# octree-nn/octfusion

Measured on AMD Instinct MI355X. Metric: denoising-steps/sec (depth-8 octree, batch 8), higher is better.
Workload: dtype f32 storage, fp16x3 products (fp16 hi + lo operand pairs = 22 significand bits, three fp16 MFMAs per product, fp32 accumulate)

## Files before the change

octfusion_amd/csrc/ofx_gemm.hip:

```cpp
#include "ofx_gemm_common.h"

constexpr int BM = 128;
constexpr int BK = 32;
constexpr int A_LD = BK + 4;
constexpr int MODE_DENSE = 0;
constexpr int MODE_GATHER = 1;

struct TileCoords { int split, tm, tn; };
__device__ __forceinline__ TileCoords tile_coords(const GemmArgs& g) {
  const int ntile = g.ntm * g.ntn;
  int bid = ofx_xcd_swizzle(blockIdx.x, ntile * g.nsplit);
  const int split = bid / ntile;
  bid -= split * ntile;
  const int tm = bid / g.ntn;
  return {split, tm, bid - tm * g.ntn};
}

__device__ __forceinline__ void load_a_dense(const GemmArgs& g, int64_t m0, int64_t k0, float4 (&va)[4]) {
  const int c4 = threadIdx.x & 7, r0 = threadIdx.x >> 3;
  const int64_t k = k0 + c4 * 4;
  const bool vec = ((g.lda & 3) == 0) && (k + 3 < g.K) && ((((uintptr_t)g.A) & 15) == 0);
#pragma unroll
  for (int i = 0; i < 4; ++i) {
    const int64_t m = m0 + r0 + 32 * i;
// ... 389 lines not shown
  const int tpd = MODE == MODE_DENSE ? nkt_all : g.cin / BK;
  const int nkt_g = MODE == MODE_DENSE ? nkt_all : ndir * tpd;
  const int g_begin = kt_begin < nkt_g ? kt_begin : nkt_g;
  const int g_end = kt_end < nkt_g ? kt_end : nkt_g;
  const int t_begin = kt_begin > nkt_g ? kt_begin : nkt_g;

  int64_t m_0 = m0 + r0, m_1 = m_0 + 32, m_2 = m_0 + 64, m_3 = m_0 + 96;
  const int64_t mmax = g.M - 1;
  m_0 = m_0 < mmax ? m_0 : mmax; m_1 = m_1 < mmax ? m_1 : mmax;
  m_2 = m_2 < mmax ? m_2 : mmax; m_3 = m_3 < mmax ? m_3 : mmax;
  const gip t0 = tab + m_0 * ndir;
  const gip t1 = tab + m_1 * ndir;
  const gip t2 = tab + m_2 * ndir;
  const gip t3 = tab + m_3 * ndir;
  int64_t dr0 = m_0, dr1 = m_1, dr2 = m_2, dr3 = m_3;
  if (MODE == MODE_DENSE && g.a_rows) { dr0 = g.a_rows[m_0]; dr1 = g.a_rows[m_1]; dr2 = g.a_rows[m_2]; dr3 = g.a_rows[m_3]; }
  const gfp dp0 = xp + dr0 * ldx, dp1 = xp + dr1 * ldx, dp2 = xp + dr2 * ldx, dp3 = xp + dr3 * ldx;
  const int kclamp = (int)g.K - 4;

  int64_t bcol[NI];
#pragma unroll
  for (int j = 0; j < NI; ++j) {
    int64_t nn = n0 + (wn * NI + j) * 32 + l31;
    bcol[j] = (nn < Ncols ? nn : Ncols - 1) + (int64_t)h * Ncols;
  }
  char* const a_st = smem8 + (r0 * 80 + c4 * 8);
  const char* const a_ld = smem8 + ((wm * MI * 32 + l31) * 80 + 16 * h);

  struct BFrag { u32x4 h[2][NI], l[2][NI]; };
  struct RegSet { float4 a0, a1, a2, a3; };
  struct IdxSet { uint32_t i0, i1, i2, i3; };

  auto load_bfrag = [&](int ktw, BFrag& F) {
    const gqp wk = w16 + (int64_t)ktw * 4 * Ncols;
#pragma unroll
    for (int c = 0; c < 2; ++c)
#pragma unroll
      for (int j = 0; j < NI; ++j) {
        F.h[c][j] = wk[(int64_t)(2 * c) * Ncols + bcol[j]];
        F.l[c][j] = wk[lo_off + (int64_t)(2 * c) * Ncols + bcol[j]];
      }
  };
  auto store_a = [&](int buf, const RegSet& R) {
    char* a = a_st + buf * BUF_BYTES;
    uint2 hi, lo;
    split16x4<H16>(R.a0, hi, lo);
    *reinterpret_cast<uint2*>(a) = hi; *reinterpret_cast<uint2*>(a + A_BYTES) = lo;
    split16x4<H16>(R.a1, hi, lo);
    *reinterpret_cast<uint2*>(a + 32 * 80) = hi; *reinterpret_cast<uint2*>(a + 32 * 80 + A_BYTES) = lo;
    split16x4<H16>(R.a2, hi, lo);
    *reinterpret_cast<uint2*>(a + 64 * 80) = hi; *reinterpret_cast<uint2*>(a + 64 * 80 + A_BYTES) = lo;
    split16x4<H16>(R.a3, hi, lo);
    *reinterpret_cast<uint2*>(a + 96 * 80) = hi; *reinterpret_cast<uint2*>(a + 96 * 80 + A_BYTES) = lo;
  };
  auto compute = [&](int buf, const BFrag& F) {
    const char* a = a_ld + buf * BUF_BYTES;
    u32x4h ah[2][MI], al[2][MI];
#pragma unroll
    for (int c = 0; c < 2; ++c)
#pragma unroll
      for (int i = 0; i < MI; ++i) {
        ah[c][i] = *reinterpret_cast<const u32x4h*>(a + i * 32 * 80 + 32 * c);
        al[c][i] = *reinterpret_cast<const u32x4h*>(a + i * 32 * 80 + 32 * c + A_BYTES);
      }
#pragma unroll
    for (int c = 0; c < 2; ++c) {
#pragma unroll
      for (int i = 0; i < MI; ++i)
#pragma unroll
        for (int j = 0; j < NI; ++j)
          acc[i][j] = mfma16<H16>(al[c][i], F.h[c][j], acc[i][j]);
#pragma unroll
      for (int i = 0; i < MI; ++i)
#pragma unroll
        for (int j = 0; j < NI; ++j)
          acc[i][j] = mfma16<H16>(ah[c][i], F.l[c][j], acc[i][j]);
#pragma unroll
      for (int i = 0; i < MI; ++i)
#pragma unroll
        for (int j = 0; j < NI; ++j)
          acc[i][j] = mfma16<H16>(ah[c][i], F.h[c][j], acc[i][j]);
    }
  };

  if (g_begin < g_end) {
    RegSet R0, R1;
    IdxSet I0 = {0, 0, 0, 0}, I1 = {0, 0, 0, 0};
    BFrag F0, F1;
    auto clampg = [&](int it) { return it < nkt_g ? it : nkt_g - 1; };
    auto ktw_of = [&](int it) {
      const int itc = clampg(it);
      return MODE == MODE_DENSE ? itc : (itc % ndir) * tpd + itc / ndir;
    };
    auto load_idx = [&](int it, IdxSet& I) {
      if (MODE == MODE_DENSE) return;
      const int dc = clampg(it) % ndir;
      I.i0 = (uint32_t)t0[dc]; I.i1 = (uint32_t)t1[dc]; I.i2 = (uint32_t)t2[dc]; I.i3 = (uint32_t)t3[dc];
    };
    auto load_rows = [&](int it, const IdxSet& I, RegSet& R) {
      const int itc = clampg(it);
      if (MODE == MODE_DENSE) {
        int cc = itc * BK + c4 * 4;
        cc = cc < kclamp ? cc : kclamp;
        R.a0 = ldg4(dp0 + cc); R.a1 = ldg4(dp1 + cc); R.a2 = ldg4(dp2 + cc); R.a3 = ldg4(dp3 + cc);
      } else {
        const int cc = (itc / ndir) * BK + c4 * 4;
        R.a0 = ldg4(xp + src_off(I.i0, ldx, n_src, aux_delta) + cc);
        R.a1 = ldg4(xp + src_off(I.i1, ldx, n_src, aux_delta) + cc);
        R.a2 = ldg4(xp + src_off(I.i2, ldx, n_src, aux_delta) + cc);
        R.a3 = ldg4(xp + src_off(I.i3, ldx, n_src, aux_delta) + cc);
      }
    };
    auto load_bchunk = [&](int ktw, int c, BFrag& F) {
      const gqp wk = w16 + (int64_t)ktw * 4 * Ncols + (int64_t)(2 * c) * Ncols;
#pragma unroll
      for (int j = 0; j < NI; ++j) { F.h[c][j] = wk[bcol[j]]; F.l[c][j] = wk[lo_off + bcol[j]]; }
    };
    auto store_half = [&](int buf, const float4& v0, const float4& v1, int row_off) {
      char* a = a_st + buf * BUF_BYTES + row_off * 80;
      uint2 hi, lo;
      split16x4<H16>(v0, hi, lo);
      *reinterpret_cast<uint2*>(a) = hi; *reinterpret_cast<uint2*>(a + A_BYTES) = lo;
      split16x4<H16>(v1, hi, lo);
      *reinterpret_cast<uint2*>(a + 32 * 80) = hi; *reinterpret_cast<uint2*>(a + 32 * 80 + A_BYTES) = lo;
    };
#define OFX_FENCE() __builtin_amdgcn_sched_barrier(0)
    auto step = [&](int it, int buf, const IdxSet& Iuse, IdxSet& Iload, const BFrag& Fcur, BFrag& Fnext,
                    RegSet& Rnew, const RegSet& Rold) {
      const char* a = a_ld + buf * BUF_BYTES;
      const int ktw = ktw_of(it + 1);
      u32x4h ah[2][MI], al[2][MI];
#pragma unroll
      for (int c = 0; c < 2; ++c)
#pragma unroll
        for (int i = 0; i < MI; ++i) {
          ah[c][i] = *reinterpret_cast<const u32x4h*>(a + i * 32 * 80 + 32 * c);
          al[c][i] = *reinterpret_cast<const u32x4h*>(a + i * 32 * 80 + 32 * c + A_BYTES);
        }
      load_idx(it + 3, Iload);
      OFX_FENCE();
#define OFX_MFMA_GROUP(AOP, BOP, C)                                                                        \
      _Pragma("unroll") for (int i = 0; i < MI; ++i)                                                        \
        _Pragma("unroll") for (int j = 0; j < NI; ++j)                                                      \
          acc[i][j] = mfma16<H16>(AOP[C][i], Fcur.BOP[C][j], acc[i][j]);
      OFX_MFMA_GROUP(al, h, 0);
      OFX_FENCE();
      load_bchunk(ktw, 0, Fnext);
      OFX_FENCE();
      OFX_MFMA_GROUP(ah, l, 0);
      OFX_FENCE();
      load_bchunk(ktw, 1, Fnext);
      OFX_FENCE();
      OFX_MFMA_GROUP(ah, h, 0);
      OFX_FENCE();
      load_rows(it + 2, Iuse, Rnew);
      OFX_FENCE();
      OFX_MFMA_GROUP(al, h, 1);
      OFX_FENCE();
      store_half(buf ^ 1, Rold.a0, Rold.a1, 0);
      OFX_FENCE();
      OFX_MFMA_GROUP(ah, l, 1);
      OFX_FENCE();
      store_half(buf ^ 1, Rold.a2, Rold.a3, 64);
      OFX_FENCE();
      OFX_MFMA_GROUP(ah, h, 1);
#undef OFX_MFMA_GROUP
      __syncthreads();
    };

    load_idx(g_begin, I0);
    load_idx(g_begin + 1, I1);
    OFX_FENCE();
    load_rows(g_begin, I0, R0);
    load_bchunk(ktw_of(g_begin), 0, F0);
    load_bchunk(ktw_of(g_begin), 1, F0);
    OFX_FENCE();
    load_idx(g_begin + 2, I0);
    OFX_FENCE();
    load_rows(g_begin + 1, I1, R1);
    OFX_FENCE();
    store_half(0, R0.a0, R0.a1, 0);
    store_half(0, R0.a2, R0.a3, 64);
    __syncthreads();
    int it = g_begin;
    for (; it + 1 < g_end; it += 2) {
      step(it, 0, I0, I1, F0, F1, R0, R1);
      step(it + 1, 1, I1, I0, F1, F0, R1, R0);
    }
    if (it < g_end) step(it, 0, I0, I1, F0, F1, R0, R1);
    __syncthreads();
#undef OFX_FENCE
  }

  for (int kt = t_begin; kt < kt_end; ++kt) {
    const int cc = (kt - nkt_g) * BK + c4 * 4;
    RegSet R;
    BFrag F;
    R.a0 = ldg4(tfp + m_0 * ldt + cc);
    R.a1 = ldg4(tfp + m_1 * ldt + cc);
    R.a2 = ldg4(tfp + m_2 * ldt + cc);
    R.a3 = ldg4(tfp + m_3 * ldt + cc);
    load_bfrag(kt, F);
    store_a(0, R);
    __syncthreads();
    compute(0, F);
    __syncthreads();
  }

  epilogue_store<WM, WN, MI, NI>(g, acc, m0, n0, wm, wn, l31, h, split);
}

__device__ __forceinline__ uint32_t bf16_rne_bits(float f) {
  const uint32_t u = __float_as_uint(f);
  return (u + 0x7fffu + ((u >> 16) & 1u)) >> 16;
}
__global__ void pack_bf16x3_kernel(const float* __restrict__ Wp, int64_t Kp, int64_t N, uint16_t* __restrict__ W16,
                                   int h16) {
  const int64_t total = Kp * N;
  const float wscale = h16 ? reinterpret_cast<const float*>(W16 + 2 * total)[1] : 1.f;
  for (int64_t t = (int64_t)blockIdx.x * blockDim.x + threadIdx.x; t < total; t += (int64_t)gridDim.x * blockDim.x) {
    const int64_t kg = t / (N * 8), rem = t - kg * N * 8;
    const int64_t n = rem / 8;
    const int kk = (int)(rem - n * 8);
    const int64_t k = kg * 8 + kk;
    const float w = Wp[((k >> 2) * N + n) * 4 + (k & 3)];
    if (h16) {
      const float ws = g2_sat16(w * wscale);
      const _Float16 hi = (_Float16)ws;
      const _Float16 lo = (_Float16)(ws - (float)hi);
      W16[t] = __builtin_bit_cast(unsigned short, hi);
      W16[total + t] = __builtin_bit_cast(unsigned short, lo);
    } else {
      const uint32_t hi = bf16_rne_bits(w);
      const float wl = w - __uint_as_float(hi << 16);
      W16[t] = (uint16_t)hi;
      W16[total + t] = (uint16_t)bf16_rne_bits(wl);
    }
  }
}
static int g_precision = 3;
static int pack_bf16x3(const float* Wp, int64_t Kp, int64_t N, hipStream_t st) {
  uint16_t* W16 = reinterpret_cast<uint16_t*>(const_cast<float*>(Wp) + Kp * N);
  if (ofx_launch_weight_scale(Wp, 1, 0, Kp * N, 1, g_precision == 3 ? 1 : 0, const_cast<float*>(Wp) + 2 * Kp * N, st))
    return OFX_ELAUNCH;
  pack_bf16x3_kernel<<<ofx_grid(Kp * N, 256), 256, 0, st>>>(Wp, Kp, N, W16, g_precision == 3 ? 1 : 0);
  return hipGetLastError() == hipSuccess ? OFX_OK : OFX_ELAUNCH;
}

extern "C" int ofx_set_precision(int mode) {
  if (mode < 0 || mode > 3) return OFX_EINVAL;
  g_precision = mode;
  return OFX_OK;
}
extern "C" int ofx_get_precision(void) { return g_precision; }
extern "C" int64_t ofx_packed_floats(int64_t Kp, int64_t N) { return 2 * Kp * N + 32; }

__global__ void __launch_bounds__(256) multi_mean_kernel(const float* __restrict__ x, int64_t ldx, int cin,
                                                         const int32_t* __restrict__ seg_ptr,
                                                         const int32_t* __restrict__ col,
                                                         const int32_t* __restrict__ multi_seg, int64_t V,
                                                         float* __restrict__ aux, int64_t ldaux,
                                                         const float* __restrict__ w) {
  const int c4n = cin >> 2;
  const int64_t total = (V + 1) * c4n;
  for (int64_t t = (int64_t)blockIdx.x * blockDim.x + threadIdx.x; t < total; t += (int64_t)gridDim.x * blockDim.x) {
    const int64_t v = t / c4n;
    const int c = (int)(t - v * c4n) * 4;
    float4 acc = f4zero();
    if (v > 0) {
      const int64_t s = multi_seg[v - 1];
      const int32_t a = seg_ptr[s], e = seg_ptr[s + 1];
      if (w) {
        for (int32_t p = a; p < e; ++p) {
          const float wp = w[p];
          const float4 xv = *reinterpret_cast<const float4*>(x + (int64_t)col[p] * ldx + c);
          acc.x += wp * xv.x; acc.y += wp * xv.y; acc.z += wp * xv.z; acc.w += wp * xv.w;
        }
      } else {
        for (int32_t p = a; p < e; ++p) f4add(acc, *reinterpret_cast<const float4*>(x + (int64_t)col[p] * ldx + c));
        const float inv = 1.f / (float)(e - a);
        acc.x *= inv; acc.y *= inv; acc.z *= inv; acc.w *= inv;
      }
    }
    *reinterpret_cast<float4*>(aux + v * ldaux + c) = acc;
  }
}

__global__ void __launch_bounds__(256) splitk_reduce_kernel(const GemmArgs g) {
  const int64_t total = g.M * g.N;
  for (int64_t t = (int64_t)blockIdx.x * blockDim.x + threadIdx.x; t < total; t += (int64_t)gridDim.x * blockDim.x) {
    const int64_t m = t / g.N, n = t - m * g.N;
    float v = 0.f;
    for (int s = 0; s < g.nsplit; ++s) v += g.ws[(int64_t)s * total + t];
    if (g.oscale_p) v *= *g.oscale_p;
    if (g.bias) v += g.bias[n];
    if (g.emb) v += g.emb[(int64_t)g.bid[m] * g.lde + n];
    if (g.res) v += g.res[m * g.ldr + n];
    int64_t om = m;
    if (g.out_rows) { om = g.out_rows[m]; if (om < 0) continue; }
    g.out[om * g.ldc + n] = v;
  }
}

__global__ void __launch_bounds__(256) splitk_reduce_v4_kernel(const GemmArgs g) {
  const int64_t n4 = g.N >> 2, total4 = g.M * n4, total = g.M * g.N;
  for (int64_t t = (int64_t)blockIdx.x * blockDim.x + threadIdx.x; t < total4; t += (int64_t)gridDim.x * blockDim.x) {
    const int64_t m = t / n4, n = (t - m * n4) * 4;
    const float* p = g.ws + m * g.N + n;
    float4 v = f4zero();
    int s = 0;
    for (; s + 7 < g.nsplit; s += 8) {
      float4 a[8];
#pragma unroll
      for (int u = 0; u < 8; ++u) a[u] = *reinterpret_cast<const float4*>(p + (int64_t)(s + u) * total);
#pragma unroll
      for (int u = 0; u < 8; ++u) f4add(v, a[u]);
    }
    for (; s + 3 < g.nsplit; s += 4) {
      const float4 a0 = *reinterpret_cast<const float4*>(p + (int64_t)s * total);
      const float4 a1 = *reinterpret_cast<const float4*>(p + (int64_t)(s + 1) * total);
      const float4 a2 = *reinterpret_cast<const float4*>(p + (int64_t)(s + 2) * total);
      const float4 a3 = *reinterpret_cast<const float4*>(p + (int64_t)(s + 3) * total);
      f4add(v, a0); f4add(v, a1); f4add(v, a2); f4add(v, a3);
    }
    for (; s < g.nsplit; ++s) f4add(v, *reinterpret_cast<const float4*>(p + (int64_t)s * total));
    if (g.oscale_p) { const float osc = *g.oscale_p; v.x *= osc; v.y *= osc; v.z *= osc; v.w *= osc; }
    if (g.bias) f4add(v, *reinterpret_cast<const float4*>(g.bias + n));
    if (g.emb) f4add(v, *reinterpret_cast<const float4*>(g.emb + (int64_t)g.bid[m] * g.lde + n));
    if (g.res) f4add(v, *reinterpret_cast<const float4*>(g.res + m * g.ldr + n));
    int64_t om = m;
    if (g.out_rows) { om = g.out_rows[m]; if (om < 0) continue; }
    if (g.out_planes) ofx_store_planes4(g.out, om * g.ldc + n, v, g.out_planes);
    else *reinterpret_cast<float4*>(g.out + om * g.ldc + n) = v;
  }
}

template <void (*KERNEL)(const GemmArgs), size_t LDS>
static int launch_tiled(GemmArgs& g, hipStream_t st) {
  static bool attr_set[OFX_MAX_DEVICES] = {};
  if (LDS > 64 * 1024 &&
      !ofx_raise_lds_limit(reinterpret_cast<const void*>(KERNEL), (int)LDS, attr_set))
    return OFX_ELAUNCH;
  KERNEL<<<g.ntm * g.ntn * g.nsplit, 256, LDS, st>>>(g);
  return OFX_OK;
}
template <int MODE, int WM, int WN, int MI, int NI>
static int launch_cfg(GemmArgs& g, int flavour, hipStream_t st) {
  constexpr size_t lds_f32 = (2 * BM * A_LD + 2 * 8 * (WN * NI * 32) * 4) * sizeof(float);
  constexpr size_t lds_16 = 2 * (2 * BM * 80);
  switch (flavour) {
    case 3: return launch_tiled<gemm_pairs_x3_kernel<MODE, WM, WN, MI, NI, 1>, lds_16>(g, st);
    case 2: return launch_tiled<gemm_pairs_x3_kernel<MODE, WM, WN, MI, NI, 0>, lds_16>(g, st);
    case 1: return launch_tiled<gemm_fast_kernel<MODE, WM, WN, MI, NI>, lds_f32>(g, st);
  }
  if constexpr (MODE == MODE_DENSE) return launch_tiled<gemm_dense_generic_kernel<WM, WN, MI, NI>, lds_f32>(g, st);
  return OFX_EINVAL;
}

__global__ void __launch_bounds__(256) stats_reduce_kernel(const float* __restrict__ part, int64_t nwr, int wr_rows,
                                                            int64_t N, const int32_t* __restrict__ bid,
                                                            double* __restrict__ stats, int64_t stats_ld) {
  __shared__ double red[3][64][2];
  const int c = threadIdx.x & 63, rg = threadIdx.x >> 6;
  const int64_t n = (int64_t)blockIdx.y * 64 + c;
  const int64_t w0 = (int64_t)blockIdx.x * 64;
  const int64_t nc = n < N ? n : N - 1;
  int b[16];
  float2 v[16];
#pragma unroll
  for (int i = 0; i < 16; ++i) {
    const int64_t w = w0 + rg * 16 + i;
    const int64_t wc = w < nwr ? w : nwr - 1;
    b[i] = bid[wc * wr_rows];
    v[i] = *reinterpret_cast<const float2*>(part + (wc * N + nc) * 2);
    if (w >= nwr) { b[i] = -1; v[i] = make_float2(0.f, 0.f); }
  }
  const int bfirst = bid[w0 * wr_rows];
  bool ok = true;
#pragma unroll
  for (int i = 0; i < 16; ++i) ok = ok && (b[i] == bfirst || b[i] < 0);
  const bool uni = __syncthreads_and(ok);
  auto flush = [&](int bb, double s, double q) {
    double* o = stats + ((int64_t)bb * stats_ld + n) * 2;
    unsafeAtomicAdd(o, s); unsafeAtomicAdd(o + 1, q);
  };
  if (uni) {
    double s = 0.0, q = 0.0;
#pragma unroll
    for (int i = 0; i < 16; ++i) { s += (double)v[i].x; q += (double)v[i].y; }
    if (rg > 0) { red[rg - 1][c][0] = s; red[rg - 1][c][1] = q; }
    __syncthreads();
    if (rg == 0 && n < N) {
#pragma unroll
      for (int r = 0; r < 3; ++r) { s += red[r][c][0]; q += red[r][c][1]; }
      flush(bfirst, s, q);
    }
  } else if (n < N) {
    double s = 0.0, q = 0.0;
    int sb = -1;
#pragma unroll
    for (int i = 0; i < 16; ++i) {
      if (b[i] < 0) continue;
      if (b[i] != sb) {
        if (sb >= 0) flush(sb, s, q);
        sb = b[i]; s = 0.0; q = 0.0;
      }
      s += (double)v[i].x; q += (double)v[i].y;
    }
    if (sb >= 0) flush(sb, s, q);
  }
}

int ofx_launch_stats_reduce(const GemmArgs& g, int wr_rows, hipStream_t st) {
  const int64_t nwr = ofx_cdiv(g.M, wr_rows);
  stats_reduce_kernel<<<dim3((unsigned)ofx_cdiv(nwr, 64), (unsigned)ofx_cdiv(g.N, 64)), 256, 0, st>>>(
      g.stats_part, nwr, wr_rows, g.N, g.bid, g.stats, g.stats_ld);
  OFX_LAUNCH_CHECK();
  return OFX_OK;
}

template <int MODE>
static int launch_gemm(GemmArgs& g, float* ws, size_t ws_bytes, hipStream_t st) {
  if (g.M <= 0 || g.N <= 0) return OFX_OK;
  if (MODE == MODE_GATHER && !(g.fast && g.nbr_ext && g.aux && (!g.out_rows || g.gather_out_rows))) return OFX_EINVAL;
  {
    auto al16 = [](const void* p) { return (reinterpret_cast<uintptr_t>(p) & 15) == 0; };
    g.vec4 = g.N % 4 == 0 && al16(g.out) && g.ldc % 4 == 0 && (!g.res || (al16(g.res) && g.ldr % 4 == 0)) &&
             (!g.emb || (al16(g.emb) && g.lde % 4 == 0)) && (!g.bias || al16(g.bias));
  }
  const int bn = g.N <= 32 ? 32 : (g.N <= 64 ? 64 : 128);
  g.ntm = (int)ofx_cdiv(g.M, BM);
  g.ntn = (int)ofx_cdiv(g.N, bn);
  const int nkt = (int)(g.Kp / BK);
  int nsplit = 1;
  const int tiles = g.ntm * g.ntn;
  if (ws && tiles < 256 && nkt >= 8) {
    nsplit = (int)ofx_cdiv(512, tiles);
    if (nsplit > nkt / 4) nsplit = nkt / 4;
    if (nsplit > 64) nsplit = 64;
    const size_t per = (size_t)g.M * g.N * sizeof(float);
    if ((size_t)nsplit * per > ws_bytes) nsplit = (int)(ws_bytes / per);
    if (nsplit < 2) nsplit = 1;
  }
  g.kt_per_split = (int)ofx_cdiv(nkt, nsplit);
  nsplit = (int)ofx_cdiv(nkt, g.kt_per_split);
  g.nsplit = nsplit;
  g.ws = ws;
  bool fast = true;
  if (MODE == MODE_DENSE) {
    fast = ((g.lda & 3) == 0) && ((g.K & 3) == 0) && g.K >= 4 && ((((uintptr_t)g.A) & 15) == 0);
    if (fast) { g.ndir = 1; g.n_src = 0; g.aux = g.A; g.tf = g.A; g.ldt = g.lda; g.nbr_ext = (const int32_t*)g.A; }
  }
  g.W16 = (g_precision != 1) ? reinterpret_cast<const uint16_t*>(g.Wp + g.Kp * g.N) : nullptr;
  const int wr_rows = bn == 32 ? 32 : 64;
  const int64_t nwr = ofx_cdiv(g.M, wr_rows);
  if (!(g.stats && g.vec4 && nsplit == 1 && g.stats_part &&
        (size_t)nwr * g.N * 2 * sizeof(float) <= g.stats_part_bytes && (((uintptr_t)g.stats_part) & 15) == 0))
    g.stats_part = nullptr;
  g.oscale_p = (fast && g.W16) ? g.Wp + 2 * g.Kp * g.N : nullptr;
  const int flavour = !fast ? 0 : (!g.W16 ? 1 : (g_precision == 3 ? 3 : 2));
  int rc;
  if (bn == 32) rc = launch_cfg<MODE, 4, 1, 1, 1>(g, flavour, st);
  else if (bn == 64) rc = launch_cfg<MODE, 2, 2, 2, 1>(g, flavour, st);
  else rc = launch_cfg<MODE, 2, 2, 2, 2>(g, flavour, st);
  if (rc) return rc;
  if (nsplit > 1) {
    const bool ws16 = (((uintptr_t)g.ws) & 15) == 0;
    if (g.vec4 && ws16) splitk_reduce_v4_kernel<<<ofx_grid(g.M * (g.N >> 2), 256), 256, 0, st>>>(g);
    else splitk_reduce_kernel<<<ofx_grid(g.M * g.N, 256), 256, 0, st>>>(g);
  }
  if (g.stats_part) {
    rc = ofx_launch_stats_reduce(g, wr_rows, st);
    if (rc) return rc;
  }
  OFX_LAUNCH_CHECK();
  return OFX_OK;
}

static inline int64_t pad32(int64_t v) { return (v + 31) / 32 * 32; }

extern "C" int64_t ofx_packed_k(int64_t K) { return pad32(K); }
extern "C" int64_t ofx_graphconv_packed_k(int cin, int nt) {
  return pad32(7 * (int64_t)cin) + (nt > 1 ? pad32(7 * (int64_t)nt) : 0);
}

__global__ void pack_weights_kernel(const float* __restrict__ W, int64_t sk, int64_t sn, int64_t K, int64_t N, int cin,
                                    int nt, float* __restrict__ Wp, int64_t Kp) {
  const int64_t total = (Kp / 4) * N;
  const int ntc = nt > 1 ? nt : 0;
  const int64_t Kf = (7 * (int64_t)cin + 31) / 32 * 32;
  for (int64_t t = (int64_t)blockIdx.x * blockDim.x + threadIdx.x; t < total; t += (int64_t)gridDim.x * blockDim.x) {
    const int64_t kq = t / N, n = t - kq * N;
    float v[4];
#pragma unroll
    for (int kk = 0; kk < 4; ++kk) {
      const int64_t k = kq * 4 + kk;
      int64_t src = -1;
      if (cin > 0) {
        if (k < 7 * (int64_t)cin) {
          const int64_t dir = k / cin, c = k - dir * cin;
          src = dir * (cin + ntc) + c;
        } else if (k >= Kf && ntc > 0 && k - Kf < 7 * (int64_t)ntc) {
          const int64_t kt = k - Kf, dir = kt / ntc, ty = kt - dir * ntc;
          src = dir * (cin + ntc) + cin + ty;
        }
      } else if (k < K) {
        src = k;
      }
      v[kk] = src >= 0 ? W[src * sk + n * sn] : 0.f;
    }
    *reinterpret_cast<float4*>(Wp + t * 4) = make_float4(v[0], v[1], v[2], v[3]);
  }
}

extern "C" int ofx_pack_weights(const float* W, int64_t sk, int64_t sn, int64_t K, int64_t N, int cin, int nt,
                                float* Wp, int64_t Kp, void* stream) {
  if (!W || !Wp || K < 1 || N < 1 || (Kp & 31) || cin < 0 || nt < 0) return OFX_EINVAL;
  if (cin > 0) {
    if (Kp != ofx_graphconv_packed_k(cin, nt) || K != 7 * (int64_t)(cin + (nt > 1 ? nt : 0))) return OFX_EINVAL;
  } else if (Kp != pad32(K)) {
    return OFX_EINVAL;
  }
  if (((uintptr_t)Wp & 15) != 0) return OFX_EINVAL;
  pack_weights_kernel<<<ofx_grid((Kp / 4) * N, 256), 256, 0, ofx_stream(stream)>>>(W, sk, sn, K, N, cin, nt, Wp, Kp);
  if (int rc = pack_bf16x3(Wp, Kp, N, ofx_stream(stream))) return rc;
  OFX_LAUNCH_CHECK();
  return OFX_OK;
}

__global__ void pack_conv3d_kernel(const float* __restrict__ W, int cin, int64_t N, float* __restrict__ Wp, int64_t Kp) {
  const int64_t total = (Kp / 4) * N;
  for (int64_t t = (int64_t)blockIdx.x * blockDim.x + threadIdx.x; t < total; t += (int64_t)gridDim.x * blockDim.x) {
    const int64_t kq = t / N, n = t - kq * N;
    float v[4];
#pragma unroll
    for (int kk = 0; kk < 4; ++kk) {
      const int64_t k = kq * 4 + kk;
      float w = 0.f;
      if (k < 27 * (int64_t)cin) {
        const int64_t tap = k / cin, c = k - tap * cin;
        w = W[(n * cin + c) * 27 + tap];
      }
      v[kk] = w;
    }
    *reinterpret_cast<float4*>(Wp + t * 4) = make_float4(v[0], v[1], v[2], v[3]);
  }
}

extern "C" int64_t ofx_conv3d_packed_k(int cin) { return pad32(27 * (int64_t)cin); }

extern "C" int ofx_pack_conv3d(const float* W, int cin, int cout, float* Wp, void* stream) {
  if (!W || !Wp || cin < 1 || cout < 1 || ((uintptr_t)Wp & 15)) return OFX_EINVAL;
  const int64_t Kp = ofx_conv3d_packed_k(cin);
  pack_conv3d_kernel<<<ofx_grid((Kp / 4) * cout, 256), 256, 0, ofx_stream(stream)>>>(W, cin, cout, Wp, Kp);
  if (int rc = pack_bf16x3(Wp, Kp, cout, ofx_stream(stream))) return rc;
  OFX_LAUNCH_CHECK();
  return OFX_OK;
}

extern "C" int ofx_gemm_f32_planes(const float* A, int64_t lda, const int32_t* a_rows, int64_t M, int64_t K,
                                   const float* Wp, int64_t Kp, int64_t N, const float* bias, const float* res, int64_t ldr,
                                   float* out, int64_t ldc, const int32_t* out_rows, void* ws, size_t ws_bytes,
                                   int out_mode, void* stream) {
  if (M == 0 && K >= 1 && N >= 1) return OFX_OK;
  if (M < 0 || K < 1 || N < 1 || !Wp || !out || (M > 0 && !A) || Kp != pad32(K) || lda < K || ldc < N ||
      (res && ldr < N) || ((uintptr_t)Wp & 15))
    return OFX_EINVAL;
  if (out_mode != 0 && out_mode != 2 && out_mode != 3) return OFX_EINVAL;
  if (out_mode && ((N & 3) || (ldc & 31) || ((uintptr_t)out & 127) || (res && ((ldr & 3) || ((uintptr_t)res & 15))) ||
                   (bias && ((uintptr_t)bias & 15)) || ((uintptr_t)ws & 15)))
    return OFX_EINVAL;
  GemmArgs g = {};
  g.A = A; g.lda = lda; g.a_rows = a_rows;
  g.M = M; g.K = K; g.Wp = Wp; g.Kp = Kp; g.N = N; g.bias = bias;
  g.res = res; g.ldr = ldr; g.out = out; g.ldc = ldc; g.out_rows = out_rows; g.out_planes = out_mode;
  return launch_gemm<MODE_DENSE>(g, (float*)ws, ws_bytes, ofx_stream(stream));
}
extern "C" int ofx_gemm_f32(const float* A, int64_t lda, const int32_t* a_rows, int64_t M, int64_t K, const float* Wp,
                            int64_t Kp, int64_t N, const float* bias, const float* res, int64_t ldr, float* out,
                            int64_t ldc, const int32_t* out_rows, void* ws, size_t ws_bytes, void* stream) {
  return ofx_gemm_f32_planes(A, lda, a_rows, M, K, Wp, Kp, N, bias, res, ldr, out, ldc, out_rows, ws, ws_bytes, 0, stream);
}

static int gather_common(GemmArgs& g, const float* x, int64_t ldx, int cin, int ndir, int64_t n_rows,
                         const int32_t* nbr, const int32_t* seg_ptr, const int32_t* col, const float* Wp, int64_t Kp,
                         int cout, const float* bias, const float* emb, int64_t lde, const int32_t* batch_id,
                         const float* res, int64_t ldr, float* out, int64_t ldc) {
  if (n_rows < 0 || cin < 1 || cout < 1 || !x || !nbr || !Wp || !out || ldx < cin || ldc < cout ||
      (res && ldr < cout) || (emb && (!batch_id || lde < cout)) || ((uintptr_t)Wp & 15))
    return OFX_EINVAL;
  g.x = x; g.ldx = ldx; g.cin = cin; g.ndir = ndir;
  g.fast = (cin % 32 == 0) && ((ldx & 3) == 0) && (((uintptr_t)x & 15) == 0);
  g.nbr = nbr; g.seg_ptr = seg_ptr; g.col = col;
  g.Kf = pad32((int64_t)ndir * cin);
  g.M = n_rows; g.K = Kp; g.Wp = Wp; g.Kp = Kp; g.N = cout; g.bias = bias;
  g.emb = emb; g.lde = lde; g.bid = batch_id; g.res = res; g.ldr = ldr; g.out = out; g.ldc = ldc;
  return OFX_OK;
}

__device__ __forceinline__ float gather_elem(const GemmArgs& g, int64_t row, int64_t k) {
  if (k >= (int64_t)g.ndir * g.cin) return 0.f;
  const int dir = (int)(k / g.cin), c = (int)(k - (int64_t)dir * g.cin);
  const int32_t nb = g.nbr[row * g.ndir + dir];
  if (nb >= 0) return g.x[(int64_t)nb * g.ldx + c];
  if (nb == -1) return 0.f;
  const int64_t s = row * g.ndir + dir;
  const int32_t a = g.seg_ptr[s], e = g.seg_ptr[s + 1];
  float acc = 0.f;
  if (g.edge_w) {
    for (int32_t p = a; p < e; ++p) acc += g.edge_w[p] * g.x[(int64_t)g.col[p] * g.ldx + c];
    return acc;
  }
  for (int32_t p = a; p < e; ++p) acc += g.x[(int64_t)g.col[p] * g.ldx + c];
  if (e - a > 1) acc /= (float)(e - a);
  return acc;
}
__global__ void __launch_bounds__(256) col_rows_kernel(const GemmArgs g, int64_t row0, int64_t rows,
                                                       float* __restrict__ colbuf) {
  const int64_t k4n = g.Kp >> 2, total = rows * k4n;
  for (int64_t t = (int64_t)blockIdx.x * blockDim.x + threadIdx.x; t < total; t += (int64_t)gridDim.x * blockDim.x) {
    const int64_t r = t / k4n, k = (t - r * k4n) * 4;
    const int64_t row = row0 + r;
    float v[4];
#pragma unroll
    for (int kk = 0; kk < 4; ++kk)
      v[kk] = (k + kk < g.Kf) ? gather_elem(g, row, k + kk) : g.tf[row * g.ldt + (k + kk - g.Kf)];
    *reinterpret_cast<float4*>(colbuf + t * 4) = make_float4(v[0], v[1], v[2], v[3]);
  }
}

static int launch_gather_via_col(const GemmArgs& g, float* ws, size_t ws_bytes, hipStream_t st) {
  if (!ws || (((uintptr_t)ws) & 15)) return OFX_EINVAL;
  size_t tail = ws_bytes / 8;
  if (tail > (size_t(16) << 20)) tail = size_t(16) << 20;
  tail &= ~size_t(15);
  const size_t row_bytes = (size_t)g.Kp * sizeof(float);
  int64_t chunk = (int64_t)((ws_bytes - tail) / row_bytes) / 128 * 128;
  if (chunk < 128) return OFX_EINVAL;
  float* tail_ws = reinterpret_cast<float*>(reinterpret_cast<char*>(ws) + (ws_bytes - tail));
  for (int64_t r0 = 0; r0 < g.M; r0 += chunk) {
    const int64_t rows = g.M - r0 < chunk ? g.M - r0 : chunk;
    col_rows_kernel<<<ofx_grid(rows * (g.Kp >> 2), 256), 256, 0, st>>>(g, r0, rows, ws);
    GemmArgs d = {};
    d.A = ws; d.lda = g.Kp; d.M = rows; d.K = g.Kp; d.Wp = g.Wp; d.Kp = g.Kp; d.N = g.N; d.bias = g.bias;
    d.emb = g.emb; d.lde = g.lde; d.bid = g.bid ? g.bid + r0 : nullptr;
    d.res = g.res ? g.res + r0 * g.ldr : nullptr; d.ldr = g.ldr;
    d.out = g.out + r0 * g.ldc; d.ldc = g.ldc;
    d.stats = g.stats; d.stats_ld = g.stats_ld;
    if (g.stats) { d.stats_part = tail_ws; d.stats_part_bytes = tail; }
    const int rc = launch_gemm<MODE_DENSE>(d, g.stats ? nullptr : tail_ws, tail, st);
    if (rc) return rc;
  }
  return OFX_OK;
}

extern "C" int ofx_graphconv_fwd(const float* x, int64_t ldx, int cin, int64_t n_nodes, const int32_t* nbr,
                                 const int32_t* seg_ptr, const int32_t* col, const int32_t* nbr_ext,
                                 const int32_t* multi_seg, int64_t n_multi, float* aux, const float* type_frac,
                                 int64_t ldt, int nt_pad, const float* Wp, int64_t Kp, int cout, const float* bias,
                                 const float* emb, int64_t lde, const int32_t* batch_id, const float* res, int64_t ldr,
                                 float* out, int64_t ldc, double* stats, int64_t stats_ld, void* ws, size_t ws_bytes,
                                 void* stream) {
  if (n_nodes == 0 && cin >= 1 && cout >= 1) return OFX_OK;
  GemmArgs g = {};
  int rc = gather_common(g, x, ldx, cin, 7, n_nodes, nbr, seg_ptr, col, Wp, Kp, cout, bias, emb, lde, batch_id, res,
                         ldr, out, ldc);
  if (rc) return rc;
  if (!seg_ptr || !col) return OFX_EINVAL;
  if (nt_pad < 0 || (nt_pad & 31) || Kp != g.Kf + nt_pad) return OFX_EINVAL;
  if (nt_pad > 0 && (!type_frac || ldt < nt_pad || (ldt & 3) || ((uintptr_t)type_frac & 15))) return OFX_EINVAL;
  g.tf = type_frac; g.ldt = ldt;
  if (stats) {
    if (!batch_id || stats_ld < cout) return OFX_EINVAL;
    g.stats = stats; g.stats_ld = stats_ld; g.bid = batch_id;
    g.stats_part = (float*)ws; g.stats_part_bytes = ws_bytes;
    ws = nullptr;
  }
  hipStream_t st = ofx_stream(stream);
  if (g.fast && nbr_ext && aux && (((uintptr_t)aux & 15) == 0)) {
    if (n_multi < 0 || (n_multi > 0 && !multi_seg)) return OFX_EINVAL;
    multi_mean_kernel<<<ofx_grid((n_multi + 1) * (cin / 4), 256), 256, 0, st>>>(x, ldx, cin, seg_ptr, col, multi_seg,
                                                                               n_multi, aux, ldx, nullptr);
    g.nbr_ext = nbr_ext; g.aux = aux; g.ldaux = ldx; g.n_src = n_nodes;
    if (!g.tf) { g.tf = x; g.ldt = ldx; }
    return launch_gemm<MODE_GATHER>(g, (float*)ws, ws_bytes, st);
  }
  return launch_gather_via_col(g, stats ? g.stats_part : (float*)ws, stats ? g.stats_part_bytes : ws_bytes, st);
}

extern "C" int ofx_graphconv_bwd_data(const float* dy, int64_t ldy, int cout, int64_t n_nodes, const int32_t* nbr_rev,
                                      const int32_t* rev_ptr, const int32_t* rev_row, const float* rev_w,
                                      const int32_t* nbr_ext_rev, const int32_t* multi_seg, int64_t n_multi, float* aux,
                                      const float* WpT, int64_t KpT, int cin, float* dx, int64_t ldx, void* ws,
                                      size_t ws_bytes, void* stream) {
  if (n_nodes == 0 && cin >= 1 && cout >= 1) return OFX_OK;
  GemmArgs g = {};
  int rc = gather_common(g, dy, ldy, cout, 7, n_nodes, nbr_rev, rev_ptr, rev_row, WpT, KpT, cin, nullptr, nullptr, 0,
                         nullptr, nullptr, 0, dx, ldx);
  if (rc) return rc;
  if (!rev_ptr || !rev_row || !rev_w || KpT != g.Kf) return OFX_EINVAL;
  g.edge_w = rev_w;
  g.tf = dy; g.ldt = ldy;
  hipStream_t st = ofx_stream(stream);
  if (g.fast && nbr_ext_rev && aux && (((uintptr_t)aux & 15) == 0)) {
    if (n_multi < 0 || (n_multi > 0 && !multi_seg)) return OFX_EINVAL;
    multi_mean_kernel<<<ofx_grid((n_multi + 1) * (cout / 4), 256), 256, 0, st>>>(dy, ldy, cout, rev_ptr, rev_row,
                                                                                multi_seg, n_multi, aux, ldy, rev_w);
    g.nbr_ext = nbr_ext_rev; g.aux = aux; g.ldaux = ldy; g.n_src = n_nodes;
    return launch_gemm<MODE_GATHER>(g, (float*)ws, ws_bytes, st);
  }
  return launch_gather_via_col(g, (float*)ws, ws_bytes, st);
}

struct TnArgs {
  const float* P; int64_t ldp;
  const float* x; int64_t ldx; int cin; int ndir;
  const int32_t* nbr_ext; const float* aux; int64_t n_src;
  const float* tf; int64_t ldt; int64_t Kf;
  const float* Q; int64_t ldq;
  int64_t rows, row0, Kp, N;
  int64_t rows_per_slice;
  float* part;
};

template <bool DENSE_P, bool BF16X3>
__global__ void __launch_bounds__(256, 2) tn_gemm_kernel(const TnArgs a) {
  constexpr int LD = 132;
  constexpr int TP = 128 * 80;
  __shared__ __attribute__((aligned(16))) char tn_smem[BF16X3 ? 4 * TP : 2 * 32 * LD * 4];
  float* const Ps = reinterpret_cast<float*>(tn_smem);
  float* const Qs = Ps + 32 * LD;
  char* const Pt = tn_smem;
  char* const Qt = tn_smem + 2 * TP;
  const int lane = threadIdx.x & 63, wid = threadIdx.x >> 6;
  const int wm = wid >> 1, wn = wid & 1, l31 = lane & 31, h = lane >> 5;
  const int64_t m0 = (int64_t)blockIdx.x * 128, n0 = (int64_t)blockIdx.y * 128;
  const int64_t r_begin = (int64_t)blockIdx.z * a.rows_per_slice;
  const int64_t r_end = r_begin + a.rows_per_slice < a.rows ? r_begin + a.rows_per_slice : a.rows;
  f32x16 acc[2][2];
#pragma unroll
  for (int i = 0; i < 2; ++i)
#pragma unroll
    for (int j = 0; j < 2; ++j)
#pragma unroll
      for (int r = 0; r < 16; ++r) acc[i][j][r] = 0.f;
  const int q4 = threadIdx.x & 3;
  const int kr = BF16X3 ? q4 + 4 * (threadIdx.x >> 5) : threadIdx.x >> 3;
  const int f0 = BF16X3 ? (threadIdx.x >> 2) & 7 : threadIdx.x & 7;
  float4 vp[4], vq[4];
  auto load_tile = [&](int64_t r) {
    const int64_t row = r + kr;
    const bool rok = row < r_end;
#pragma unroll
    for (int p = 0; p < 4; ++p) {
      const int64_t m = m0 + 4 * (f0 + 8 * p), n = n0 + 4 * (f0 + 8 * p);
      float4 v = f4zero();
      if (rok && m < a.Kp) {
        if (DENSE_P) {
          v = *reinterpret_cast<const float4*>(a.P + row * a.ldp + m);
        } else if (m < a.Kf) {
          const int64_t kk = m;
          if (kk < a.ndir * (int64_t)a.cin) {
            const int dir = (int)(kk / a.cin), c = (int)(kk - (int64_t)dir * a.cin);
            const int64_t id = a.nbr_ext[(a.row0 + row) * a.ndir + dir];
            const float* src = id < a.n_src ? a.x + id * a.ldx : a.aux + (id - a.n_src) * a.ldx;
            v = *reinterpret_cast<const float4*>(src + c);
          }
        } else {
          v = *reinterpret_cast<const float4*>(a.tf + (a.row0 + row) * a.ldt + (m - a.Kf));
        }
      }
      vp[p] = v;
// ... 376 lines not shown
```

octfusion_amd/csrc/ofx_gemm_common.h:

```cpp
#pragma once
#include "ofx_common.h"

typedef float f32x16 __attribute__((ext_vector_type(16)));

struct GemmArgs {
  const float* A; int64_t lda; const int32_t* a_rows;
  const float* x; int64_t ldx; int cin; int ndir; int fast;
  const int32_t* nbr;
  const int32_t* seg_ptr; const int32_t* col;
  const float* edge_w;
  const float* tf; int64_t ldt; int64_t Kf;
  const int32_t* nbr_ext;
  const float* aux; int64_t ldaux; int64_t n_src;
  int64_t M, K;
  const float* Wp; int64_t Kp, N;
  const uint16_t* W16;
  const float* oscale_p;
  const float* bias;
  const float* emb; int64_t lde; const int32_t* bid;
  const float* res; int64_t ldr;
  float* out; int64_t ldc; const int32_t* out_rows;
  int gather_out_rows;
  int out_planes;
  double* stats; int64_t stats_ld;
  int ntm, ntn, nsplit, kt_per_split;
  float* ws;
  int vec4;
  float* stats_part; size_t stats_part_bytes;
};

static __global__ void __launch_bounds__(256) weight_absmax_kernel(const float* __restrict__ W, int64_t sk, int64_t sn, int64_t K,
                                                            int64_t N, unsigned* __restrict__ acc) {
  __shared__ float red[256];
  float m = 0.f;
  for (int64_t t = (int64_t)blockIdx.x * 256 + threadIdx.x; t < K * N; t += (int64_t)gridDim.x * 256) {
    const float a = fabsf(W[(t / N) * sk + (t % N) * sn]);
    if (a <= 3.0e38f) m = fmaxf(m, a);
  }
  red[threadIdx.x] = m;
  __syncthreads();
  for (int o = 128; o > 0; o >>= 1) {
    if ((int)threadIdx.x < o) red[threadIdx.x] = fmaxf(red[threadIdx.x], red[threadIdx.x + o]);
    __syncthreads();
  }
  if (threadIdx.x == 0) atomicMax(acc, __float_as_uint(red[0]));
}
static __global__ void weight_scale_finish_kernel(int fp16_operands, float* __restrict__ scale) {
  const float mx = __uint_as_float(reinterpret_cast<const unsigned*>(scale)[0]);
  float s = 1.f;
  if (fp16_operands && mx > 0.f) {
    int e;
    frexpf(mx, &e);
    int sh = 15 - e;
    sh = sh < -60 ? -60 : (sh > 60 ? 60 : sh);
    s = ldexpf(1.f, sh);
  }
  scale[0] = 1.f / s;
  scale[1] = s;
}
static inline int ofx_launch_weight_scale(const float* W, int64_t sk, int64_t sn, int64_t K, int64_t N, int fp16_operands,
                                          float* scale, hipStream_t st) {
  if (hipMemsetAsync(scale, 0, sizeof(float), st) != hipSuccess) return OFX_ELAUNCH;
  int64_t nb = (K * N + 256 * 16 - 1) / (256 * 16);
  nb = nb < 1 ? 1 : (nb > 1024 ? 1024 : nb);
  weight_absmax_kernel<<<(unsigned)nb, 256, 0, st>>>(W, sk, sn, K, N, reinterpret_cast<unsigned*>(scale));
  if (hipGetLastError() != hipSuccess) return OFX_ELAUNCH;
  weight_scale_finish_kernel<<<1, 1, 0, st>>>(fp16_operands, scale);
  if (hipGetLastError() != hipSuccess) return OFX_ELAUNCH;
  return OFX_OK;
}


__device__ __forceinline__ unsigned g2_pk_bf16(float a, float b) {
  unsigned r;
  asm("v_cvt_pk_bf16_f32 %0, %1, %2" : "=v"(r) : "v"(a), "v"(b));
  return r;
}
__device__ __forceinline__ unsigned g2_pk_f16(float a, float b) {
  const _Float16 x = (_Float16)a, y = (_Float16)b;
  return (unsigned)__builtin_bit_cast(unsigned short, x) | ((unsigned)__builtin_bit_cast(unsigned short, y) << 16);
}
__device__ __forceinline__ float g2_bf16_lo(unsigned p) { return __uint_as_float(p << 16); }
__device__ __forceinline__ float g2_bf16_hi(unsigned p) { return __uint_as_float(p & 0xffff0000u); }
__device__ __forceinline__ float g2_f16_lo(unsigned p) { return (float)__builtin_bit_cast(_Float16, (unsigned short)(p & 0xffffu)); }
__device__ __forceinline__ float g2_f16_hi(unsigned p) { return (float)__builtin_bit_cast(_Float16, (unsigned short)(p >> 16)); }
__device__ __forceinline__ float g2_sat16(float v) { return fminf(fmaxf(v, -65504.f), 65504.f); }
__device__ __forceinline__ void g2_split2(int mode, float a, float b, unsigned& hi, unsigned& lo) {
  if (mode == 3) {
    hi = g2_pk_f16(a, b);
    lo = g2_pk_f16(a - g2_f16_lo(hi), b - g2_f16_hi(hi));
  } else {
    hi = g2_pk_bf16(a, b);
    lo = g2_pk_bf16(a - g2_bf16_lo(hi), b - g2_bf16_hi(hi));
  }
}
__device__ __forceinline__ void g2_join2(int mode, unsigned hi, unsigned lo, float& a, float& b) {
  if (mode == 3) { a = g2_f16_lo(hi) + g2_f16_lo(lo); b = g2_f16_hi(hi) + g2_f16_hi(lo); }
  else { a = g2_bf16_lo(hi) + g2_bf16_lo(lo); b = g2_bf16_hi(hi) + g2_bf16_hi(lo); }
}
__host__ __device__ static inline bool g2_pairs(int mode) { return mode == 2 || mode == 3; }

__device__ __forceinline__ void ofx_store_planes4(float* base, int64_t f, const float4& v, int mode) {
  unsigned h0, h1, l0, l1;
  g2_split2(mode, v.x, v.y, h0, l0);
  g2_split2(mode, v.z, v.w, h1, l1);
  char* o = reinterpret_cast<char*>(base) + (f >> 5) * 128 + (f & 31) * 2;
  *reinterpret_cast<uint2*>(o) = make_uint2(h0, h1);
  *reinterpret_cast<uint2*>(o + 64) = make_uint2(l0, l1);
}

__device__ __forceinline__ int ofx_xcd_swizzle(int bid, int n) {
  const int q = n / 8, r = n % 8, xcd = bid % 8, j = bid / 8;
  return (xcd < r ? xcd * (q + 1) : r * (q + 1) + (xcd - r) * q) + j;
}

__device__ __forceinline__ float4 f4zero() { return make_float4(0.f, 0.f, 0.f, 0.f); }
__device__ __forceinline__ void f4add(float4& a, const float4& b) { a.x += b.x; a.y += b.y; a.z += b.z; a.w += b.w; }

template <int WM, int WN, int MI, int NI>
__device__ __forceinline__ void epilogue_store_scalar(const GemmArgs& g, f32x16 (&acc)[MI][NI], int64_t m0, int64_t n0,
                                                      int wm, int wn, int l31, int h, int split) {
#pragma unroll
  for (int j = 0; j < NI; ++j) {
    const int64_t n = n0 + (wn * NI + j) * 32 + l31;
    if (n >= g.N) continue;
    if (g.nsplit > 1) {
#pragma unroll
      for (int i = 0; i < MI; ++i)
#pragma unroll
        for (int r = 0; r < 16; ++r) {
          const int64_t m = m0 + (wm * MI + i) * 32 + (r & 3) + 8 * (r >> 2) + 4 * h;
          if (m < g.M) g.ws[((int64_t)split * g.M + m) * g.N + n] = acc[i][j][r];
        }
      continue;
    }
    const float bv = g.bias ? g.bias[n] : 0.f;
    const float osc = g.oscale_p ? *g.oscale_p : 1.f;
    int sb = -1;
    float ssum = 0.f, ssq = 0.f;
#pragma unroll
    for (int i = 0; i < MI; ++i) {
#pragma unroll
      for (int r = 0; r < 16; ++r) {
        const int64_t m = m0 + (wm * MI + i) * 32 + (r & 3) + 8 * (r >> 2) + 4 * h;
        if (m >= g.M) continue;
        float v = fmaf(acc[i][j][r], osc, bv);
        int b = 0;
        if (g.emb || g.stats) b = g.bid[m];
        if (g.emb) v += g.emb[(int64_t)b * g.lde + n];
        if (g.res) v += g.res[m * g.ldr + n];
        if (g.stats) {
          if (b != sb) {
            if (sb >= 0) {
              double* o = g.stats + ((int64_t)sb * g.stats_ld + n) * 2;
              unsafeAtomicAdd(o, (double)ssum);
              unsafeAtomicAdd(o + 1, (double)ssq);
            }
            sb = b; ssum = 0.f; ssq = 0.f;
          }
          ssum += v; ssq += v * v;
        }
        int64_t om = m;
        if (g.out_rows) { om = g.out_rows[m]; if (om < 0) continue; }
        g.out[om * g.ldc + n] = v;
      }
    }
    if (g.stats && sb >= 0) {
      double* o = g.stats + ((int64_t)sb * g.stats_ld + n) * 2;
      unsafeAtomicAdd(o, (double)ssum);
      unsafeAtomicAdd(o + 1, (double)ssq);
    }
  }
}

__device__ __forceinline__ float dpp_xor1(float v) {
  return __builtin_bit_cast(float, __builtin_amdgcn_mov_dpp(__builtin_bit_cast(int, v), 0xB1, 0xf, 0xf, true));
}
__device__ __forceinline__ float dpp_xor2(float v) {
  return __builtin_bit_cast(float, __builtin_amdgcn_mov_dpp(__builtin_bit_cast(int, v), 0x4E, 0xf, 0xf, true));
}
__device__ __forceinline__ void quad_transpose(float& v0, float& v1, float& v2, float& v3, bool q0, bool q1) {
  float r = dpp_xor1(q0 ? v0 : v1);
  if (q0) v0 = r; else v1 = r;
  r = dpp_xor1(q0 ? v2 : v3);
  if (q0) v2 = r; else v3 = r;
  r = dpp_xor2(q1 ? v0 : v2);
  if (q1) v0 = r; else v2 = r;
  r = dpp_xor2(q1 ? v1 : v3);
  if (q1) v1 = r; else v3 = r;
}

template <int WM, int WN, int MI, int NI>
__device__ __forceinline__ void epilogue_store_v4(const GemmArgs& g, f32x16 (&acc)[MI][NI], int64_t m0, int64_t n0,
                                                  int wm, int wn, int l31, int h) {
  const int q = l31 & 3, k = l31 >> 2;
  const bool q0 = q & 1, q1 = q & 2;
  const int64_t mw = m0 + wm * MI * 32;
  const int64_t blockIdx_tm = m0 / (WM * MI * 32);
  const float osc = g.oscale_p ? *g.oscale_p : 1.f;
  int bids[MI][4];
  bool uni = true;
  int b0 = 0;
  if (g.emb || g.stats) {
    const int64_t mlast = g.M - 1;
    b0 = g.bid[mw < mlast ? mw : mlast];
#pragma unroll
    for (int i = 0; i < MI; ++i)
#pragma unroll
      for (int G = 0; G < 4; ++G) {
        const int64_t m = mw + i * 32 + q + 4 * h + 8 * G;
        bids[i][G] = g.bid[m < mlast ? m : mlast];
        uni = uni && (bids[i][G] == b0);
      }
    uni = __all(uni);
  }
#pragma unroll
  for (int j = 0; j < NI; ++j) {
    const int64_t n = n0 + (wn * NI + j) * 32 + 4 * k;
    const bool ncol = n < g.N;
    float4 bv = f4zero();
    if (g.bias && ncol) bv = *reinterpret_cast<const float4*>(g.bias + n);
    float4 ssum = f4zero(), ssq = f4zero();
    int sb = -1;
    auto flush = [&](int b) {
      double* o = g.stats + ((int64_t)b * g.stats_ld + n) * 2;
      unsafeAtomicAdd(o + 0, (double)ssum.x); unsafeAtomicAdd(o + 1, (double)ssq.x);
      unsafeAtomicAdd(o + 2, (double)ssum.y); unsafeAtomicAdd(o + 3, (double)ssq.y);
      unsafeAtomicAdd(o + 4, (double)ssum.z); unsafeAtomicAdd(o + 5, (double)ssq.z);
      unsafeAtomicAdd(o + 6, (double)ssum.w); unsafeAtomicAdd(o + 7, (double)ssq.w);
    };
#pragma unroll
    for (int i = 0; i < MI; ++i) {
      float4 t[4];
#pragma unroll
      for (int G = 0; G < 4; ++G) {
        float v0 = acc[i][j][4 * G], v1 = acc[i][j][4 * G + 1], v2 = acc[i][j][4 * G + 2], v3 = acc[i][j][4 * G + 3];
        quad_transpose(v0, v1, v2, v3, q0, q1);
        t[G] = make_float4(fmaf(v0, osc, bv.x), fmaf(v1, osc, bv.y), fmaf(v2, osc, bv.z), fmaf(v3, osc, bv.w));
      }
#pragma unroll
      for (int G = 0; G < 4; ++G) {
        const int64_t m = mw + i * 32 + q + 4 * h + 8 * G;
        if (m >= g.M || !ncol) continue;
        float4 v = t[G];
        if (g.emb) f4add(v, *reinterpret_cast<const float4*>(g.emb + (int64_t)bids[i][G] * g.lde + n));
        if (g.res) f4add(v, *reinterpret_cast<const float4*>(g.res + m * g.ldr + n));
        if (g.stats) {
          const int b = bids[i][G];
          if (!uni && b != sb) {
            if (sb >= 0) flush(sb);
            ssum = f4zero(); ssq = f4zero();
          }
          sb = b;
          f4add(ssum, v);
          ssq.x += v.x * v.x; ssq.y += v.y * v.y; ssq.z += v.z * v.z; ssq.w += v.w * v.w;
        }
        int64_t om = m;
        if (g.out_rows) { om = g.out_rows[m]; if (om < 0) continue; }
        if (g.out_planes) ofx_store_planes4(g.out, om * g.ldc + n, v, g.out_planes);
        else *reinterpret_cast<float4*>(g.out + om * g.ldc + n) = v;
      }
    }
    if (g.stats) {
      if (uni) {
#define OFX_RED(f) f += dpp_xor1(f); f += dpp_xor2(f); f += __shfl_xor(f, 32);
        OFX_RED(ssum.x) OFX_RED(ssum.y) OFX_RED(ssum.z) OFX_RED(ssum.w)
        OFX_RED(ssq.x) OFX_RED(ssq.y) OFX_RED(ssq.z) OFX_RED(ssq.w)
#undef OFX_RED
        if (q == 0 && h == 0 && ncol && mw < g.M) {
          if (g.stats_part) {
            float* o = g.stats_part + (((int64_t)blockIdx_tm * WM + wm) * g.N + n) * 2;
            *reinterpret_cast<float4*>(o) = make_float4(ssum.x, ssq.x, ssum.y, ssq.y);
            *reinterpret_cast<float4*>(o + 4) = make_float4(ssum.z, ssq.z, ssum.w, ssq.w);
          } else {
            flush(b0);
          }
        }
      } else {
        if (sb >= 0 && ncol) flush(sb);
        if (g.stats_part && q == 0 && h == 0 && ncol && mw < g.M) {
          float* o = g.stats_part + (((int64_t)blockIdx_tm * WM + wm) * g.N + n) * 2;
          *reinterpret_cast<float4*>(o) = f4zero();
          *reinterpret_cast<float4*>(o + 4) = f4zero();
        }
      }
    }
  }
}

template <int WM, int WN, int MI, int NI>
__device__ __forceinline__ void epilogue_store(const GemmArgs& g, f32x16 (&acc)[MI][NI], int64_t m0, int64_t n0, int wm,
                                               int wn, int l31, int h, int split) {
  if (g.vec4 && g.nsplit == 1) epilogue_store_v4<WM, WN, MI, NI>(g, acc, m0, n0, wm, wn, l31, h);
  else epilogue_store_scalar<WM, WN, MI, NI>(g, acc, m0, n0, wm, wn, l31, h, split);
}
```

Before: 119.2.

## Store split-K partials in accumulator-native layout and reduce with quad transpose

Split-K GEMM partials are now written straight from the MFMA accumulator registers as contiguous float4s in a tile/wave/fragment-ordered workspace, replacing the scattered scalar stores into row-major M×N. A new templated reduce kernel reads these partials in coalesced order, transposes each quad in registers to recover row-major float4s, and applies scale, bias, embedding, residual and row remapping. This removes uncoalesced scalar epilogue stores on the split-K path. In exchange the workspace is sized per padded tile, which can lower nsplit when workspace is tight, and the reduce grid now depends on the tile configuration.

```diff
diff --git a/octfusion_amd/csrc/ofx_gemm.hip b/octfusion_amd/csrc/ofx_gemm.hip
--- a/octfusion_amd/csrc/ofx_gemm.hip
+++ b/octfusion_amd/csrc/ofx_gemm.hip
@@ -715,37 +715,50 @@
   }
 }
 
-__global__ void __launch_bounds__(256) splitk_reduce_v4_kernel(const GemmArgs g) {
-  const int64_t n4 = g.N >> 2, total4 = g.M * n4, total = g.M * g.N;
-  for (int64_t t = (int64_t)blockIdx.x * blockDim.x + threadIdx.x; t < total4; t += (int64_t)gridDim.x * blockDim.x) {
-    const int64_t m = t / n4, n = (t - m * n4) * 4;
-    const float* p = g.ws + m * g.N + n;
-    float4 v = f4zero();
-    int s = 0;
-    for (; s + 7 < g.nsplit; s += 8) {
-      float4 a[8];
-#pragma unroll
-      for (int u = 0; u < 8; ++u) a[u] = *reinterpret_cast<const float4*>(p + (int64_t)(s + u) * total);
-#pragma unroll
-      for (int u = 0; u < 8; ++u) f4add(v, a[u]);
-    }
-    for (; s + 3 < g.nsplit; s += 4) {
-      const float4 a0 = *reinterpret_cast<const float4*>(p + (int64_t)s * total);
-      const float4 a1 = *reinterpret_cast<const float4*>(p + (int64_t)(s + 1) * total);
-      const float4 a2 = *reinterpret_cast<const float4*>(p + (int64_t)(s + 2) * total);
-      const float4 a3 = *reinterpret_cast<const float4*>(p + (int64_t)(s + 3) * total);
-      f4add(v, a0); f4add(v, a1); f4add(v, a2); f4add(v, a3);
-    }
-    for (; s < g.nsplit; ++s) f4add(v, *reinterpret_cast<const float4*>(p + (int64_t)s * total));
-    if (g.oscale_p) { const float osc = *g.oscale_p; v.x *= osc; v.y *= osc; v.z *= osc; v.w *= osc; }
-    if (g.bias) f4add(v, *reinterpret_cast<const float4*>(g.bias + n));
-    if (g.emb) f4add(v, *reinterpret_cast<const float4*>(g.emb + (int64_t)g.bid[m] * g.lde + n));
-    if (g.res) f4add(v, *reinterpret_cast<const float4*>(g.res + m * g.ldr + n));
-    int64_t om = m;
-    if (g.out_rows) { om = g.out_rows[m]; if (om < 0) continue; }
-    if (g.out_planes) ofx_store_planes4(g.out, om * g.ldc + n, v, g.out_planes);
-    else *reinterpret_cast<float4*>(g.out + om * g.ldc + n) = v;
-  }
+template <int WM, int WN, int MI, int NI>
+__global__ void __launch_bounds__(256) splitk_reduce_acc_kernel(const GemmArgs g) {
+  constexpr int UPW = MI * NI * 4;
+  const int lane = threadIdx.x & 63;
+  const int l31 = lane & 31, h = lane >> 5, q = l31 & 3, k = l31 >> 2;
+  const int64_t u = (int64_t)blockIdx.x * 4 + (threadIdx.x >> 6);
+  const int G = (int)(u & 3), ij = (int)((u >> 2) % (MI * NI));
+  const int64_t pw = u / UPW;
+  const int wave = (int)(pw % (WM * WN));
+  const int64_t tile = pw / (WM * WN);
+  const int64_t tm = tile / g.ntn, tn = tile - tm * g.ntn;
+  const int64_t m8 = tm * BM + ((wave / WN) * MI + ij / NI) * 32 + 8 * G;
+  const int64_t n32 = tn * (WN * NI * 32) + ((wave % WN) * NI + ij % NI) * 32;
+  if (m8 >= g.M || n32 >= g.N) return;
+  const int64_t slice = (int64_t)g.ntm * g.ntn * (BM * WN * NI * 32);
+  const float* p = g.ws + (u * 64 + lane) * 4;
+  float4 v = f4zero();
+  int s = 0;
+  for (; s + 7 < g.nsplit; s += 8) {
+    float4 a[8];
+#pragma unroll
+    for (int t = 0; t < 8; ++t) a[t] = *reinterpret_cast<const float4*>(p + (int64_t)(s + t) * slice);
+#pragma unroll
+    for (int t = 0; t < 8; ++t) f4add(v, a[t]);
+  }
+  for (; s + 3 < g.nsplit; s += 4) {
+    const float4 a0 = *reinterpret_cast<const float4*>(p + (int64_t)s * slice);
+    const float4 a1 = *reinterpret_cast<const float4*>(p + (int64_t)(s + 1) * slice);
+    const float4 a2 = *reinterpret_cast<const float4*>(p + (int64_t)(s + 2) * slice);
+    const float4 a3 = *reinterpret_cast<const float4*>(p + (int64_t)(s + 3) * slice);
+    f4add(v, a0); f4add(v, a1); f4add(v, a2); f4add(v, a3);
+  }
+  for (; s < g.nsplit; ++s) f4add(v, *reinterpret_cast<const float4*>(p + (int64_t)s * slice));
+  quad_transpose(v.x, v.y, v.z, v.w, q & 1, q & 2);
+  const int64_t m = m8 + q + 4 * h, n = n32 + 4 * k;
+  if (m >= g.M || n >= g.N) return;
+  if (g.oscale_p) { const float osc = *g.oscale_p; v.x *= osc; v.y *= osc; v.z *= osc; v.w *= osc; }
+  if (g.bias) f4add(v, *reinterpret_cast<const float4*>(g.bias + n));
+  if (g.emb) f4add(v, *reinterpret_cast<const float4*>(g.emb + (int64_t)g.bid[m] * g.lde + n));
+  if (g.res) f4add(v, *reinterpret_cast<const float4*>(g.res + m * g.ldr + n));
+  int64_t om = m;
+  if (g.out_rows) { om = g.out_rows[m]; if (om < 0) return; }
+  if (g.out_planes) ofx_store_planes4(g.out, om * g.ldc + n, v, g.out_planes);
+  else *reinterpret_cast<float4*>(g.out + om * g.ldc + n) = v;
 }
 
 template <void (*KERNEL)(const GemmArgs), size_t LDS>
@@ -846,12 +859,14 @@
   g.ntn = (int)ofx_cdiv(g.N, bn);
   const int nkt = (int)(g.Kp / BK);
   int nsplit = 1;
+  bool ws_acc = false;
   const int tiles = g.ntm * g.ntn;
   if (ws && tiles < 256 && nkt >= 8) {
     nsplit = (int)ofx_cdiv(512, tiles);
     if (nsplit > nkt / 4) nsplit = nkt / 4;
     if (nsplit > 64) nsplit = 64;
-    const size_t per = (size_t)g.M * g.N * sizeof(float);
+    ws_acc = g.vec4 && (((uintptr_t)ws) & 15) == 0;
+    const size_t per = (ws_acc ? (size_t)tiles * BM * bn : (size_t)g.M * g.N) * sizeof(float);
     if ((size_t)nsplit * per > ws_bytes) nsplit = (int)(ws_bytes / per);
     if (nsplit < 2) nsplit = 1;
   }
@@ -859,6 +874,7 @@
   nsplit = (int)ofx_cdiv(nkt, g.kt_per_split);
   g.nsplit = nsplit;
   g.ws = ws;
+  g.ws_acc = nsplit > 1 && ws_acc;
   bool fast = true;
   if (MODE == MODE_DENSE) {
     fast = ((g.lda & 3) == 0) && ((g.K & 3) == 0) && g.K >= 4 && ((((uintptr_t)g.A) & 15) == 0);
@@ -878,9 +894,11 @@
   else rc = launch_cfg<MODE, 2, 2, 2, 2>(g, flavour, st);
   if (rc) return rc;
   if (nsplit > 1) {
-    const bool ws16 = (((uintptr_t)g.ws) & 15) == 0;
-    if (g.vec4 && ws16) splitk_reduce_v4_kernel<<<ofx_grid(g.M * (g.N >> 2), 256), 256, 0, st>>>(g);
-    else splitk_reduce_kernel<<<ofx_grid(g.M * g.N, 256), 256, 0, st>>>(g);
+    const unsigned nb = (unsigned)tiles * (BM * bn / 1024);
+    if (!g.ws_acc) splitk_reduce_kernel<<<ofx_grid(g.M * g.N, 256), 256, 0, st>>>(g);
+    else if (bn == 32) splitk_reduce_acc_kernel<4, 1, 1, 1><<<nb, 256, 0, st>>>(g);
+    else if (bn == 64) splitk_reduce_acc_kernel<2, 2, 2, 1><<<nb, 256, 0, st>>>(g);
+    else splitk_reduce_acc_kernel<2, 2, 2, 2><<<nb, 256, 0, st>>>(g);
   }
   if (g.stats_part) {
     rc = ofx_launch_stats_reduce(g, wr_rows, st);
diff --git a/octfusion_amd/csrc/ofx_gemm_common.h b/octfusion_amd/csrc/ofx_gemm_common.h
--- a/octfusion_amd/csrc/ofx_gemm_common.h
+++ b/octfusion_amd/csrc/ofx_gemm_common.h
@@ -26,6 +26,7 @@
   int ntm, ntn, nsplit, kt_per_split;
   float* ws;
   int vec4;
+  int ws_acc;
   float* stats_part; size_t stats_part_bytes;
 };
 
@@ -289,8 +290,25 @@
 }
 
 template <int WM, int WN, int MI, int NI>
+__device__ __forceinline__ void epilogue_store_partials(const GemmArgs& g, f32x16 (&acc)[MI][NI], int64_t m0, int64_t n0,
+                                                        int wm, int wn, int l31, int h, int split) {
+  const int64_t tile = m0 / (WM * MI * 32) * g.ntn + n0 / (WN * NI * 32);
+  float* p = g.ws + ((((int64_t)split * g.ntm * g.ntn + tile) * (WM * WN) + wm * WN + wn) * (MI * NI * 4) * 64 +
+                     l31 + 32 * h) * 4;
+#pragma unroll
+  for (int i = 0; i < MI; ++i)
+#pragma unroll
+    for (int j = 0; j < NI; ++j)
+#pragma unroll
+      for (int G = 0; G < 4; ++G)
+        *reinterpret_cast<float4*>(p + ((i * NI + j) * 4 + G) * 256) =
+            make_float4(acc[i][j][4 * G], acc[i][j][4 * G + 1], acc[i][j][4 * G + 2], acc[i][j][4 * G + 3]);
+}
+
+template <int WM, int WN, int MI, int NI>
 __device__ __forceinline__ void epilogue_store(const GemmArgs& g, f32x16 (&acc)[MI][NI], int64_t m0, int64_t n0, int wm,
                                                int wn, int l31, int h, int split) {
-  if (g.vec4 && g.nsplit == 1) epilogue_store_v4<WM, WN, MI, NI>(g, acc, m0, n0, wm, wn, l31, h);
+  if (g.ws_acc) epilogue_store_partials<WM, WN, MI, NI>(g, acc, m0, n0, wm, wn, l31, h, split);
+  else if (g.vec4 && g.nsplit == 1) epilogue_store_v4<WM, WN, MI, NI>(g, acc, m0, n0, wm, wn, l31, h);
   else epilogue_store_scalar<WM, WN, MI, NI>(g, acc, m0, n0, wm, wn, l31, h, split);
 }
```

Result: no change. 120.0 (median of 6 runs) (+0.6%).
